# moble/scri

Measured on AMD Instinct MI355X. Metric: timesteps/sec for full BMS transform, l_max=16, 1e5 steps; fp64, higher is better.
Workload: dtype f64

## Files before the change

scri_amd/csrc/kernels_gemm_eval.hip:

```cpp
#include <cstdio>
#include <cstdlib>
#include <vector>

#include "kernels.h"

namespace bms {

typedef double v4d __attribute__((ext_vector_type(4)));

constexpr int E_BM = 64, E_BN = 64, E_KC = 8;
constexpr int E_PA = 10;
constexpr int E_PB = 64;
constexpr int E_ASZ = E_BM * E_PA;
constexpr int E_BSZ = E_KC * E_PB;
constexpr int E_PC = 33;

struct EvalArgs {
  const BsplineTable* table;
  const double* x;
  const double* skew_a;
  const double* skew_b;
  double tt;
  long long g0, n, i_lo, i_hi;
  double* out;
  long long ldo;
  int search_halfwidth;
  double inv_dx;
  double* side;
  long long side_ld;
  unsigned long long* stats;
  int dbg;
  unsigned long long* trace;
};

#if BMS_PROBES
#define EV_DBG(ev) ((ev).dbg)
#define EV_TRACE(ev) ((ev).trace)
#else
#define EV_DBG(ev) 0
#define EV_TRACE(ev) (static_cast<unsigned long long*>(nullptr))
#endif

__device__ __forceinline__ int eval_lower_bound(const double* __restrict__ bp, int n_i, double sa, double sb, double tt, double y,
                                                long long guess, int halfwidth) {
  auto ue = [&](int i) {
    const double xi = bp[i];
    return xi + (sa * (xi - tt) + sb);
  };
  int lo = 0, hi = n_i;
  if (halfwidth > 0) {
    long long a = guess - halfwidth, b = guess + halfwidth;
    if (a < 0) a = 0;
    if (b > n_i) b = n_i;
    if (a < b) {
      const bool ok_lo = (a == 0) || ue((int)a - 1) < y;
      const bool ok_hi = (b == n_i) || !(ue((int)b) < y);
      if (ok_lo && ok_hi) lo = (int)a, hi = (int)b;
    }
  }
  while (lo < hi) {
    const int mid = (lo + hi) >> 1;
    if (ue(mid) < y)
      lo = mid + 1;
    else
      hi = mid;
  }
  return lo;
}

__device__ __forceinline__ double2 eval_ld2(const double* p) { return *reinterpret_cast<const double2*>(p); }
__device__ __forceinline__ double2 eval_ld2(const double __attribute__((address_space(3))) * p) {
  typedef double v2d_t __attribute__((ext_vector_type(2)));
  const v2d_t v = *(const v2d_t __attribute__((address_space(3)))*)p;
  return double2{v.x, v.y};
}

struct EvalMarch {
  int jl, jl_end, jl_open, f_lo, f_hi, i, n_i;
  double sa, sb, tt;
  double* op;
  long long ldo;
};

template <bool INTERIOR, class SRC, class WIN>
__device__ __forceinline__ bool eval_march(EvalMarch& m, const SRC& src, WIN win, int dbg) {
  if (!src.has(m.i)) return false;
  double xi = src.samp(m.i);
  double sk = m.sa * (xi - m.tt) + m.sb;
  double ue = xi + sk;
  const double inf = __builtin_huge_val();
  double xhi = (!INTERIOR && m.jl >= m.jl_open) ? inf : src.knot(m.jl + 1);
  while (true) {
    if (!(ue < xhi)) {
      if (++m.jl >= m.jl_end) return true;
      xhi = (!INTERIOR && m.jl >= m.jl_open) ? inf : src.knot(m.jl + 1);
    }
    if (ue < xhi) {
      const auto tb = src.tab(m.jl);
      int fl = m.jl - 1;
      if (!INTERIOR) fl = fl < m.f_lo ? m.f_lo : (fl > m.f_hi ? m.f_hi : fl);
      const double2 q0 = win(fl, 0), q1 = win(fl, 1), q2 = win(fl, 2), q3 = win(fl, 3);
      const double t = (xi - src.knot(m.jl)) + sk;
      const double2 m0 = eval_ld2(tb + 0), m1 = eval_ld2(tb + 2), m2 = eval_ld2(tb + 4), m3 = eval_ld2(tb + 6);
      const double2 m4 = eval_ld2(tb + 8), m5 = eval_ld2(tb + 10), m6 = eval_ld2(tb + 12), m7 = eval_ld2(tb + 14);
      const double b0 = fma(fma(fma(m6.x, t, m4.x), t, m2.x), t, m0.x);
      const double b1 = fma(fma(fma(m6.y, t, m4.y), t, m2.y), t, m0.y);
      const double b2 = fma(fma(fma(m7.x, t, m5.x), t, m3.x), t, m1.x);
      const double b3 = fma(fma(fma(m7.y, t, m5.y), t, m3.y), t, m1.y);
      double2 v;
      v.x = fma(b3, q3.x, fma(b2, q2.x, fma(b1, q1.x, b0 * q0.x)));
      v.y = fma(b3, q3.y, fma(b2, q2.y, fma(b1, q1.y, b0 * q0.y)));
      if (!(dbg & 2)) *reinterpret_cast<double2*>(m.op) = v;
      m.op += m.ldo;
      if (++m.i >= m.n_i) return true;
      if (!src.has(m.i)) return false;
      xi = src.samp(m.i);
      sk = m.sa * (xi - m.tt) + m.sb;
      ue = xi + sk;
    }
  }
}

struct EvalFromGlobal {
  const EvalArgs& ev;
  const double* bp;
  long long kT;
  __device__ __forceinline__ double knot(int jl) const { return ev.x[kT + jl]; }
  __device__ __forceinline__ const double* tab(int jl) const { return ev.table[kT + jl].m; }
  __device__ __forceinline__ bool has(int) const { return true; }
  __device__ __forceinline__ double samp(int i) const { return bp[i]; }
};
constexpr int E_XS = 256;
typedef const double __attribute__((address_space(3))) * lds_cdp;
typedef const double2 __attribute__((address_space(3))) * lds_cd2p;
struct EvalFromLds {
  lds_cdp t_lds;
  lds_cdp xk_lds;
  lds_cdp xs_lds;
  int i_a;
  double inv_dx;
  __device__ __forceinline__ double knot(int jl) const { return xk_lds[jl]; }
  __device__ __forceinline__ lds_cdp tab(int jl) const { return t_lds + 16 * jl; }
  __device__ __forceinline__ bool has(int i) const { return (unsigned)(i - i_a) < (unsigned)E_XS; }
  __device__ __forceinline__ double samp(int i) const { return xs_lds[i - i_a]; }
  __device__ __forceinline__ int first(double y, double sa, double sb, double tt, int n_i) const {
    int lo = 0, hi = E_XS;
    if (inv_dx > 0.0) {
      const double z = (y - (sb - sa * tt)) / (1.0 + sa);
      const double gf = (z - xs_lds[0]) * inv_dx;
      int g = gf < 0.0 ? 0 : (gf > (double)(E_XS - 1) ? E_XS - 1 : (int)gf);
      const double xa = xs_lds[g], xb = xs_lds[g + 1 < E_XS ? g + 1 : E_XS - 1];
      const bool below = xa + (sa * (xa - tt) + sb) < y;
      const bool next_below = xb + (sa * (xb - tt) + sb) < y;
      if (below && !next_below && g + 1 < E_XS)
        lo = hi = g + 1;
      else if (!below && g > 0) {
        const double xc = xs_lds[g - 1];
        if (xc + (sa * (xc - tt) + sb) < y) lo = hi = g;
      }
    }
#pragma unroll
    for (int st = 0; st < 9; ++st) {
      const int mid = lo < hi ? (lo + hi) >> 1 : (lo < E_XS ? lo : E_XS - 1);
      const double xi = xs_lds[mid];
      if (lo < hi) {
        if (xi + (sa * (xi - tt) + sb) < y)
          lo = mid + 1;
        else
          hi = mid;
      }
    }
    if ((lo > 0 || i_a == 0) && (lo < E_XS || i_a + E_XS >= n_i)) return (i_a + lo) < n_i ? (i_a + lo) : n_i;
    return -1;
  }
};

__device__ __forceinline__ bool eval_launch_wide_window(const EvalArgs& ev) {
  return !(ev.inv_dx > 0.0) || (EV_DBG(ev) & 32) || (ev.search_halfwidth > 0 && 2 * ev.search_halfwidth + 72 <= E_XS);
}
__device__ __forceinline__ bool eval_tile_window(const EvalArgs& ev, long long kT, int rows, int n_i, double smin, double smax, double inv_dx, int* i_a) {
  if (eval_launch_wide_window(ev)) {
    const bool ok = ev.search_halfwidth > 0 && 2 * ev.search_halfwidth + 72 <= E_XS;
    long long ia = kT - ev.i_lo - ev.search_halfwidth - 2;
    ia = ia > n_i - 1 ? n_i - 1 : ia;
    *i_a = (int)(ia < 0 ? 0 : ia);
    return ok;
  }
  const double r_hi = smax * inv_dx, r_lo = smin * inv_dx;
  const double amax = fabs(r_hi) > fabs(r_lo) ? fabs(r_hi) : fabs(r_lo);
  if (!(amax < 1e8)) {
    *i_a = 0;
    return false;
  }
  const long long margin = 3 + (long long)(0.03 * amax);
  long long ia = kT - ev.i_lo - (long long)ceil(r_hi) - margin - 1;
  const long long ib = kT + rows - ev.i_lo - (long long)floor(r_lo) + margin + 1;
  const bool ok = ib - ia <= E_XS;
  ia = ia > n_i - 1 ? n_i - 1 : ia;
  *i_a = (int)(ia < 0 ? 0 : ia);
  return ok;
}
__device__ __forceinline__ void wave_min_max(double& mn, double& mx) {
#pragma unroll
  for (int d = 32; d >= 1; d >>= 1) {
    const double a = __shfl_xor(mn, d, 64), b = __shfl_xor(mx, d, 64);
    mn = a < mn ? a : mn;
    mx = b > mx ? b : mx;
  }
}

template <class WIN>
__device__ __forceinline__ void eval_windows(const EvalArgs& ev, const bool from_lds, const EvalFromLds lds, int col, double sa, double sb, long long kT,
                                             int fa, int fb, WIN win) {
  const long long n = ev.n;
  {
    const long long cap = n - 3 - kT;
    if (fb > cap) fb = (int)cap;
  }
  if (fa >= fb) return;
  constexpr int FAR = 1 << 24;
  EvalMarch m;
  m.f_lo = kT > FAR ? -FAR : (int)(-kT), m.f_hi = n - 4 - kT > FAR ? FAR : (int)(n - 4 - kT);
  m.jl_open = n - 2 - kT > FAR ? FAR : (int)(n - 2 - kT);
  m.jl = fa == m.f_lo ? m.f_lo : fa + 1;
  m.jl_end = fb - 1 == m.f_hi ? m.jl_open + 1 : fb + 1;
  m.sa = sa, m.sb = sb;
  m.n_i = (int)(ev.i_hi - ev.i_lo);
  m.tt = ev.tt;
  m.ldo = ev.ldo;
  const double* bp = ev.x + ev.i_lo;
  int i = -1;
  if (kT + m.jl == 0)
    i = 0;
  else if (from_lds)
    i = lds.first(lds.knot(m.jl), m.sa, m.sb, m.tt, m.n_i);
  if (i < 0) {
    if (from_lds && ev.stats) atomicAdd(ev.stats + 1, 1ull);
    i = eval_lower_bound(bp, m.n_i, m.sa, m.sb, m.tt, ev.x[kT + m.jl], kT + m.jl - ev.i_lo, ev.search_halfwidth);
  }
  if (i >= m.n_i) return;
  m.i = i;
  m.op = ev.out + 2LL * col + (long long)i * ev.ldo;
  const bool interior = fa > m.f_lo && fb - 1 < m.f_hi && fb + 1 < m.jl_open;
  if (from_lds && interior) {
    if (eval_march<true>(m, lds, win, EV_DBG(ev))) return;
  } else if (from_lds) {
    if (eval_march<false>(m, lds, win, EV_DBG(ev))) return;
  }
  if (from_lds && ev.stats) atomicAdd(ev.stats + 1, 1ull);
  eval_march<false>(m, EvalFromGlobal{ev, bp, kT}, win, EV_DBG(ev));
}

template <int ROW_STEP>
__global__ __launch_bounds__(256, 3) void zgemm3m_eval_kernel(const double* __restrict__ A, long long lda, const double* __restrict__ B,
                                                             long long ldb, long long M, int N, int K, int nbm, int nbn,
                                                             int st_rows_log2, const double* __restrict__ col_scale, EvalArgs ev) {
  __shared__ __attribute__((aligned(16))) double2 lds[2 * E_ASZ + 2 * E_BSZ];
  static_assert(sizeof(double2) * (2 * E_ASZ + 2 * E_BSZ) >= sizeof(double2) * E_BM * E_PC, "the parked half tile must fit the operand LDS");
  __shared__ __attribute__((aligned(16))) double t_lds[64 * 16];
  __shared__ __attribute__((aligned(16))) double xk_lds[64];
  __shared__ __attribute__((aligned(16))) double xs_lds[E_XS];
  __shared__ __attribute__((aligned(16))) double2 sk_lds[E_BN];
  __shared__ double win_lds[4];
  double2* As = lds;
  double2* Bs = lds + 2 * E_ASZ;

  const int b = blockIdx.x;
  const int xcd = b & 7;
  const int q = b >> 3;
  const int st_cols_log2 = 6 - st_rows_log2;
  const int nsn = (nbn + (1 << st_cols_log2) - 1) >> st_cols_log2;
  const int S = (q >> 6) * 8 + xcd;
  const int r = q & 63;
  const int bm = ((S / nsn) << st_rows_log2) + (r >> st_cols_log2);
  const int bn = ((S % nsn) << st_cols_log2) + (r & ((1 << st_cols_log2) - 1));
  if (bm >= nbm || bn >= nbn) return;
  const long long m0 = (long long)bm * ROW_STEP;
  const int n0 = bn * E_BN;
  unsigned long long tr_t0 = 0;
  if (EV_TRACE(ev)) tr_t0 = __builtin_readcyclecounter();
  const int tid = threadIdx.x;
  const int wave = __builtin_amdgcn_readfirstlane(tid >> 6), lane = tid & 63;
  const int wm = wave >> 1, wn = wave & 1;
  const int fi = lane & 15, fk = lane >> 4;

  const long long rows_valid = (M - m0) < E_BM ? (M - m0) : E_BM;
  const long long kT = ev.g0 + m0;
  const int n_i = (int)(ev.i_hi - ev.i_lo);
  if (tid < E_BN) {
    const int col = n0 + tid < N ? n0 + tid : N - 1;
    const double sa = ev.skew_a ? ev.skew_a[col] : 0.0, sb = ev.skew_b ? ev.skew_b[col] : 0.0;
    sk_lds[tid] = double2{sa, sb};
    if (!eval_launch_wide_window(ev)) {
      const double s0 = sa * (ev.x[kT] - ev.tt) + sb, s1 = sa * (ev.x[kT + rows_valid - 1] - ev.tt) + sb;
      double mn = s0 < s1 ? s0 : s1, mx = s0 < s1 ? s1 : s0;
      wave_min_max(mn, mx);
      if (tid == 0) win_lds[0] = mn, win_lds[1] = mx;
    }
    if (tid == 0) {
      const double span = ev.x[kT + rows_valid - 1] - ev.x[kT];
      win_lds[2] = (rows_valid > 1 && span > 0.0) ? (double)(rows_valid - 1) / span : ev.inv_dx;
    }
  }

  v4d p1[2][2], p2[2][2], p3[2][2];
#pragma unroll
  for (int i = 0; i < 2; ++i)
#pragma unroll
    for (int j = 0; j < 2; ++j) p1[i][j] = p2[i][j] = p3[i][j] = v4d{0.0, 0.0, 0.0, 0.0};

  const int a_row = tid >> 3, a_k = tid & 7;
  const int b_row = tid >> 6, b_col = tid & 63;
  const double* a_ptr = A + (m0 + a_row) * lda + 2 * a_k;
  const double* b_ptr = B + (long long)b_row * ldb + 2 * (n0 + b_col);
  const bool a_ok0 = (m0 + a_row) < M, a_ok1 = (m0 + a_row + 32) < M;
  const double2 zero2 = {0.0, 0.0};
  double2 ra0, ra1, rb0, rb1;
  const int nk = (K + E_KC - 1) / E_KC;

#define E_LOAD_GLOBAL(kt)                                                                      \
  {                                                                                            \
    const int k0 = (kt)*E_KC;                                                                  \
    const bool kok = (k0 + a_k) < K;                                                           \
    ra0 = (a_ok0 && kok) ? *reinterpret_cast<const double2*>(a_ptr + 2 * k0) : zero2;          \
    ra1 = (a_ok1 && kok) ? *reinterpret_cast<const double2*>(a_ptr + 32 * lda + 2 * k0) : zero2; \
    const double* bp_ = b_ptr + (long long)k0 * ldb;                                           \
    rb0 = *reinterpret_cast<const double2*>(bp_);                                              \
    rb1 = *reinterpret_cast<const double2*>(bp_ + 4 * ldb);                                    \
  }
#define E_STORE_LDS(buf)                                        \
  {                                                             \
    double2* as_w = As + (buf)*E_ASZ + a_row * E_PA + a_k;      \
    as_w[0] = ra0;                                              \
    as_w[32 * E_PA] = ra1;                                      \
    double2* bs_w = Bs + (buf)*E_BSZ + b_row * E_PB + b_col;    \
    bs_w[0] = rb0;                                              \
    bs_w[4 * E_PB] = rb1;                                       \
  }

  E_LOAD_GLOBAL(0);
  E_STORE_LDS(0);
  __syncthreads();
  int i_a;
  const bool wide = eval_launch_wide_window(ev);
  const bool from_lds = eval_tile_window(ev, kT, (int)rows_valid, n_i, wide ? 0.0 : win_lds[0], wide ? 0.0 : win_lds[1], win_lds[2], &i_a);
  if (!from_lds && tid == 0 && ev.stats) atomicAdd(ev.stats, 1ull);
  if (from_lds) {
    if (tid == 0) {
      const int i_b = i_a + E_XS - 1 < n_i - 1 ? i_a + E_XS - 1 : n_i - 1;
      const double span = ev.x[ev.i_lo + i_b] - ev.x[ev.i_lo + i_a];
      win_lds[3] = (ev.inv_dx > 0.0 && i_b > i_a && span > 0.0) ? (double)(i_b - i_a) / span : 0.0;
    }
    {
      long long row = tid >> 2;
      if (row > rows_valid - 1) row = rows_valid - 1;
      const double* src = ev.table[kT + row].m + 4 * (tid & 3);
      const double2 v0 = *reinterpret_cast<const double2*>(src), v1 = *reinterpret_cast<const double2*>(src + 2);
      double2* dst = reinterpret_cast<double2*>(t_lds + 16 * (tid >> 2) + 4 * (tid & 3));
      dst[0] = v0, dst[1] = v1;
    }
    if (tid < 64) {
      long long row = tid;
      if (row > rows_valid - 1) row = rows_valid - 1;
      xk_lds[tid] = ev.x[kT + row];
    }
    {
      int i = i_a + tid;
      if (i > n_i - 1) i = n_i - 1;
      xs_lds[tid] = ev.x[ev.i_lo + i];
    }
  }

  const bool narrow = n0 + 32 >= N;
  const int rbase = narrow ? wave * 16 : wm * 32, cbase = narrow ? 0 : wn * 32;
  const bool wave_has_columns = n0 + cbase < N;
  for (int kt = 0; kt < nk; ++kt) {
    const int buf = kt & 1;
    if (kt + 1 < nk) E_LOAD_GLOBAL(kt + 1);
    const double2* as = As + buf * E_ASZ + (rbase + fi) * E_PA + fk;
    const double2* bs = Bs + buf * E_BSZ + fk * E_PB + cbase + fi;
#pragma unroll
    for (int kk = 0; wave_has_columns && kk < E_KC / 4; ++kk) {
      const double2 a0 = as[kk * 4];
      const double2 b0 = bs[kk * 4 * E_PB], b1 = bs[kk * 4 * E_PB + 16];
      const double sa0 = a0.x + a0.y, sb0 = b0.x + b0.y, sb1 = b1.x + b1.y;
      p1[0][0] = __builtin_amdgcn_mfma_f64_16x16x4f64(a0.x, b0.x, p1[0][0], 0, 0, 0);
      p1[0][1] = __builtin_amdgcn_mfma_f64_16x16x4f64(a0.x, b1.x, p1[0][1], 0, 0, 0);
      p2[0][0] = __builtin_amdgcn_mfma_f64_16x16x4f64(a0.y, b0.y, p2[0][0], 0, 0, 0);
      p2[0][1] = __builtin_amdgcn_mfma_f64_16x16x4f64(a0.y, b1.y, p2[0][1], 0, 0, 0);
      p3[0][0] = __builtin_amdgcn_mfma_f64_16x16x4f64(sa0, sb0, p3[0][0], 0, 0, 0);
      p3[0][1] = __builtin_amdgcn_mfma_f64_16x16x4f64(sa0, sb1, p3[0][1], 0, 0, 0);
      if (!narrow) {
        const double2 a1 = as[16 * E_PA + kk * 4];
        const double sa1 = a1.x + a1.y;
        p1[1][0] = __builtin_amdgcn_mfma_f64_16x16x4f64(a1.x, b0.x, p1[1][0], 0, 0, 0);
        p1[1][1] = __builtin_amdgcn_mfma_f64_16x16x4f64(a1.x, b1.x, p1[1][1], 0, 0, 0);
        p2[1][0] = __builtin_amdgcn_mfma_f64_16x16x4f64(a1.y, b0.y, p2[1][0], 0, 0, 0);
        p2[1][1] = __builtin_amdgcn_mfma_f64_16x16x4f64(a1.y, b1.y, p2[1][1], 0, 0, 0);
        p3[1][0] = __builtin_amdgcn_mfma_f64_16x16x4f64(sa1, sb0, p3[1][0], 0, 0, 0);
        p3[1][1] = __builtin_amdgcn_mfma_f64_16x16x4f64(sa1, sb1, p3[1][1], 0, 0, 0);
      }
    }
    if (kt + 1 < nk) E_STORE_LDS(buf ^ 1);
    __syncthreads();
  }
#undef E_LOAD_GLOBAL
#undef E_STORE_LDS

  unsigned long long tr_t1 = 0;
  if (EV_TRACE(ev)) tr_t1 = __builtin_readcyclecounter();
  double2 cv[2][2][4];
#pragma unroll
  for (int j = 0; j < 2; ++j) {
    const int col = n0 + cbase + j * 16 + fi;
    const bool okc = col < N;
    const double sc_r = (okc && col_scale) ? col_scale[2 * col] : 1.0, sc_i = (okc && col_scale) ? col_scale[2 * col + 1] : 1.0;
#pragma unroll
    for (int i = 0; i < 2; ++i)
#pragma unroll
      for (int rr = 0; rr < 4; ++rr) {
        const double re = p1[i][j][rr] - p2[i][j][rr];
        const double im = (p3[i][j][rr] - p1[i][j][rr]) - p2[i][j][rr];
        cv[i][j][rr] = double2{re * sc_r, im * sc_i};
      }
  }
  double2* Cs = lds;
  const int ec = tid & 31, eg = tid >> 5;
#pragma unroll
  for (int h = 0; h < 2; ++h) {
    if (narrow ? h == 0 : wn == h) {
#pragma unroll
      for (int j = 0; j < 2; ++j)
#pragma unroll
        for (int i = 0; i < 2; ++i)
#pragma unroll
          for (int rr = 0; rr < 4; ++rr)
            if (i == 0 || !narrow) Cs[(rbase + i * 16 + fk + 4 * rr) * E_PC + j * 16 + fi] = cv[i][j][rr];
    }
    __syncthreads();
    const int col = n0 + h * 32 + ec;
    if (col < N && !(EV_DBG(ev) & 1)) {
      if (ROW_STEP == 64 && ev.side != nullptr && eg < 6) {
        const int row = eg < 3 ? eg : 58 + eg;
        if (row < rows_valid) *reinterpret_cast<double2*>(ev.side + ((long long)bm * 6 + eg) * ev.side_ld + 2LL * col) = Cs[row * E_PC + ec];
      }
      int fa = 8 * eg, fb = fa + 8;
      const int f_own = 61, f_rows = (int)rows_valid - 3;
      if (fb > f_own) fb = f_own;
      if (fb > f_rows) fb = f_rows;
      const auto win = [&](int fl, int qq) { return Cs[(fl + qq) * E_PC + ec]; };
      const EvalFromLds src{(lds_cdp)t_lds, (lds_cdp)xk_lds, (lds_cdp)xs_lds, i_a, from_lds ? win_lds[3] : 0.0};
      const double2 sk = sk_lds[h * 32 + ec];
      eval_windows(ev, from_lds, src, col, sk.x, sk.y, kT, fa, fb, win);
    }
    if (h == 0) __syncthreads();
  }
  if (EV_TRACE(ev) && tid == 0) {
    const unsigned hw = __builtin_amdgcn_s_getreg((31 << 11) | 4), xcc = __builtin_amdgcn_s_getreg((31 << 11) | 20);
    unsigned long long* tp = ev.trace + 5LL * b;
    tp[0] = (unsigned long long)hw | ((unsigned long long)xcc << 32);
    tp[1] = (unsigned long long)bm | ((unsigned long long)bn << 32);
    tp[2] = tr_t0, tp[3] = tr_t1, tp[4] = __builtin_readcyclecounter();
  }
}

__global__ __launch_bounds__(64) void spline_straddle_eval_kernel(int N, int n_row_tiles, int n_col_panels, EvalArgs ev, long long M) {
  __shared__ __attribute__((aligned(16))) double2 w_lds[6][64];
  __shared__ __attribute__((aligned(16))) double t_lds[8 * 16];
  __shared__ __attribute__((aligned(16))) double xk_lds[8];
  __shared__ __attribute__((aligned(16))) double xs_lds[E_XS];
  const int tid = threadIdx.x;
  const int bnd = blockIdx.x / n_col_panels;
  const int col = (blockIdx.x - bnd * n_col_panels) * 64 + tid;
  if (bnd + 1 >= n_row_tiles) return;
  const long long kT = ev.g0 + 64LL * bnd + 61;
  const int n_i = (int)(ev.i_hi - ev.i_lo);
  const long long k_last = ev.g0 + M - 1;
  const int colc = col < N ? col : N - 1;
  const double sa_t = ev.skew_a ? ev.skew_a[colc] : 0.0, sb_t = ev.skew_b ? ev.skew_b[colc] : 0.0;
  double smin = 0.0, smax = 0.0;
  if (!eval_launch_wide_window(ev)) {
    const double s0 = sa_t * (ev.x[kT] - ev.tt) + sb_t, s1 = sa_t * (ev.x[kT + 5 > k_last ? k_last : kT + 5] - ev.tt) + sb_t;
    smin = s0 < s1 ? s0 : s1, smax = s0 < s1 ? s1 : s0;
    wave_min_max(smin, smax);
  }
  double inv_dx_loc = ev.inv_dx;
  {
    const long long ka = kT - 29 < ev.g0 ? ev.g0 : kT - 29, kb = kT + 34 > k_last ? k_last : kT + 34;
    const double span = ev.x[kb] - ev.x[ka];
    if (kb > ka && span > 0.0) inv_dx_loc = (double)(kb - ka) / span;
  }
  int i_a;
  const bool from_lds = eval_tile_window(ev, kT, 6, n_i, smin, smax, inv_dx_loc, &i_a);
  if (!from_lds && tid == 0 && ev.stats) atomicAdd(ev.stats, 1ull);
  double inv_dx_win = 0.0;
  if (from_lds) {
    {
      const int i_b = i_a + E_XS - 1 < n_i - 1 ? i_a + E_XS - 1 : n_i - 1;
      const double span = ev.x[ev.i_lo + i_b] - ev.x[ev.i_lo + i_a];
      if (ev.inv_dx > 0.0 && i_b > i_a && span > 0.0) inv_dx_win = (double)(i_b - i_a) / span;
    }
    {
      long long jj = kT + (tid >> 3);
      if (jj > k_last) jj = k_last;
      reinterpret_cast<double2*>(t_lds)[tid] = *reinterpret_cast<const double2*>(ev.table[jj].m + 2 * (tid & 7));
    }
    if (tid < 8) {
      long long jj = kT + tid;
      if (jj > k_last) jj = k_last;
      xk_lds[tid] = ev.x[jj];
    }
#pragma unroll
    for (int r = 0; r < E_XS / 64; ++r) {
      int i = i_a + tid + 64 * r;
      if (i > n_i - 1) i = n_i - 1;
      xs_lds[tid + 64 * r] = ev.x[ev.i_lo + i];
    }
    __syncthreads();
  }
  if (col >= N) return;
  int fb = 3;
  {
    const long long f_rows = ev.g0 + M - 3 - kT;
    if (fb > f_rows) fb = (int)f_rows;
  }
  const double* s0 = ev.side + ((long long)bnd * 6 + 3) * ev.side_ld + 2LL * col;
  const double* s1 = ev.side + ((long long)(bnd + 1) * 6 + 0) * ev.side_ld + 2LL * col;
#pragma unroll
  for (int e = 0; e < 3; ++e) {
    w_lds[e][tid] = *reinterpret_cast<const double2*>(s0 + e * ev.side_ld);
    w_lds[3 + e][tid] = *reinterpret_cast<const double2*>(s1 + e * ev.side_ld);
  }
  const auto win = [&](int fl, int qq) { return w_lds[fl + qq][tid]; };
  const EvalFromLds src{(lds_cdp)t_lds, (lds_cdp)xk_lds, (lds_cdp)xs_lds, i_a, inv_dx_win};
  eval_windows(ev, from_lds, src, col, sa_t, sb_t, kT, 0, fb, win);
}

hipError_t launch_zgemm3m_eval(hipStream_t stream, const double* A, long long lda, const double* B, long long ldb, long long M, int N,
                               int K, const double* col_scale, const SplineEval& e) {
  if (M <= 0 || N <= 0 || e.i_hi <= e.i_lo) return hipSuccess;
  if (M < 4) return hipErrorInvalidValue;
  EvalArgs ev;
  ev.table = e.table, ev.x = e.x, ev.skew_a = e.skew_a, ev.skew_b = e.skew_b, ev.tt = e.tt, ev.g0 = e.g0, ev.n = e.n_knots;
  ev.i_lo = e.i_lo, ev.i_hi = e.i_hi, ev.out = e.out, ev.ldo = e.ldo, ev.search_halfwidth = e.search_halfwidth;
  ev.inv_dx = e.inv_dx;
  ev.side = e.side, ev.side_ld = e.side_ld;
  ev.stats = e.stats;
  ev.dbg = 0;
#if BMS_PROBES
  static const int dbg_env = BMS_PROBE_ENV("SCRI_AMD_GEMM_EVAL_DBG") ? atoi(BMS_PROBE_ENV("SCRI_AMD_GEMM_EVAL_DBG")) : 0;
  ev.dbg = dbg_env;
#endif
  const int step = (e.step == 61 || e.step == 64) ? e.step : (e.side ? 64 : 61);
  if (step == 64 && !e.side) return hipErrorInvalidValue;
  if (step == 61) ev.side = nullptr;
  const int nbm = step == 61 ? (int)((M - 3 + 60) / 61) : (int)((M + 63) / 64);
  const int nbn = (N + E_BN - 1) / E_BN;
  static const int st_env = BMS_PROBE_ENV("SCRI_AMD_ZGEMM_ST_ROWS_LOG2") ? atoi(BMS_PROBE_ENV("SCRI_AMD_ZGEMM_ST_ROWS_LOG2")) : -1;
  const int st_rows_log2 = (st_env >= 0 && st_env <= 6) ? st_env : (nbm >= 512 ? 6 : 5);
  const int sr = 1 << st_rows_log2, sc = 64 >> st_rows_log2;
  const long long n_super = (long long)((nbm + sr - 1) / sr) * ((nbn + sc - 1) / sc);
  const long long grid = ((n_super + 7) / 8) * 8 * 64;
  ev.trace = nullptr;
#if BMS_PROBES
  const char* trace_path = BMS_PROBE_ENV("SCRI_AMD_GEMM_EVAL_TRACE");
  if (trace_path) {
    if (hipMalloc(&ev.trace, 40 * (size_t)grid) != hipSuccess) ev.trace = nullptr;
    if (ev.trace) (void)hipMemsetAsync(ev.trace, 0, 40 * (size_t)grid, stream);
  }
#endif
  if (step == 61)
    hipLaunchKernelGGL(zgemm3m_eval_kernel<61>, dim3((unsigned)grid), dim3(256), 0, stream, A, lda, B, ldb, M, N, K, nbm, nbn, st_rows_log2,
                       col_scale, ev);
  else {
    hipLaunchKernelGGL(zgemm3m_eval_kernel<64>, dim3((unsigned)grid), dim3(256), 0, stream, A, lda, B, ldb, M, N, K, nbm, nbn, st_rows_log2,
                       col_scale, ev);
    const long long n_straddle = (long long)(nbm - 1) * nbn;
    if (n_straddle > 0x7fffffffLL) return hipErrorInvalidValue;
    if (nbm > 1 && !(EV_DBG(ev) & 4))
      hipLaunchKernelGGL(spline_straddle_eval_kernel, dim3((unsigned)n_straddle), dim3(64), 0, stream, N, nbm, nbn, ev, M);
  }
#if BMS_PROBES
  if (ev.trace) {
    std::vector<unsigned long long> h(5 * (size_t)grid);
    (void)hipStreamSynchronize(stream);
    (void)hipMemcpy(h.data(), ev.trace, 40 * (size_t)grid, hipMemcpyDeviceToHost);
    (void)hipFree(ev.trace);
    if (FILE* f = fopen(trace_path, "wb")) {
      fwrite(h.data(), 8, h.size(), f);
      fclose(f);
    }
  }
#endif
  return hipGetLastError();
}

long long zgemm3m_eval_side_rows(long long M) { return 6 * ((M + 63) / 64); }

}
```

Measured before the change: 19.07 million.

## Micro-optimize fused zgemm-eval kernel: buffer loads, precomputed reciprocals, magic division

Bundles several micro-optimizations into the fused GEMM+spline-eval kernel. Global tile loads move to raw buffer loads with out-of-bounds zeroing in place of per-lane predicated loads, and the k-loop is unrolled by two. Per-column 1/(1+sa) is precomputed and stored in LDS, the binary search is skipped when no lane needs it (wave ballot), and the superblock div/mod uses a host-computed magic multiplier. The tile window computation moves into the prologue on thread 0 and is broadcast with readfirstlane. These changes add launch-time stride checks and rely on buffer OOB semantics being correct for the tails.

```diff
diff --git a/scri_amd/csrc/kernels_gemm_eval.hip b/scri_amd/csrc/kernels_gemm_eval.hip
--- a/scri_amd/csrc/kernels_gemm_eval.hip
+++ b/scri_amd/csrc/kernels_gemm_eval.hip
@@ -143,10 +143,10 @@
   __device__ __forceinline__ lds_cdp tab(int jl) const { return t_lds + 16 * jl; }
   __device__ __forceinline__ bool has(int i) const { return (unsigned)(i - i_a) < (unsigned)E_XS; }
   __device__ __forceinline__ double samp(int i) const { return xs_lds[i - i_a]; }
-  __device__ __forceinline__ int first(double y, double sa, double sb, double tt, int n_i) const {
+  __device__ __forceinline__ int first(double y, double sa, double sb, double tt, double rinv, int n_i) const {
     int lo = 0, hi = E_XS;
     if (inv_dx > 0.0) {
-      const double z = (y - (sb - sa * tt)) / (1.0 + sa);
+      const double z = (y - (sb - sa * tt)) * rinv;
       const double gf = (z - xs_lds[0]) * inv_dx;
       int g = gf < 0.0 ? 0 : (gf > (double)(E_XS - 1) ? E_XS - 1 : (int)gf);
       const double xa = xs_lds[g], xb = xs_lds[g + 1 < E_XS ? g + 1 : E_XS - 1];
@@ -159,15 +159,17 @@
         if (xc + (sa * (xc - tt) + sb) < y) lo = hi = g;
       }
     }
-#pragma unroll
-    for (int st = 0; st < 9; ++st) {
-      const int mid = lo < hi ? (lo + hi) >> 1 : (lo < E_XS ? lo : E_XS - 1);
-      const double xi = xs_lds[mid];
-      if (lo < hi) {
-        if (xi + (sa * (xi - tt) + sb) < y)
-          lo = mid + 1;
-        else
-          hi = mid;
+    if (__builtin_amdgcn_ballot_w64(lo < hi) != 0) {
+#pragma unroll
+      for (int st = 0; st < 9; ++st) {
+        const int mid = lo < hi ? (lo + hi) >> 1 : (lo < E_XS ? lo : E_XS - 1);
+        const double xi = xs_lds[mid];
+        if (lo < hi) {
+          if (xi + (sa * (xi - tt) + sb) < y)
+            lo = mid + 1;
+          else
+            hi = mid;
+        }
       }
     }
     if ((lo > 0 || i_a == 0) && (lo < E_XS || i_a + E_XS >= n_i)) return (i_a + lo) < n_i ? (i_a + lo) : n_i;
@@ -210,8 +212,8 @@
 }
 
 template <class WIN>
-__device__ __forceinline__ void eval_windows(const EvalArgs& ev, const bool from_lds, const EvalFromLds lds, int col, double sa, double sb, long long kT,
-                                             int fa, int fb, WIN win) {
+__device__ __forceinline__ void eval_windows(const EvalArgs& ev, const bool from_lds, const EvalFromLds lds, int col, double sa, double sb, double rinv,
+                                             long long kT, int fa, int fb, WIN win) {
   const long long n = ev.n;
   {
     const long long cap = n - 3 - kT;
@@ -233,7 +235,7 @@
   if (kT + m.jl == 0)
     i = 0;
   else if (from_lds)
-    i = lds.first(lds.knot(m.jl), m.sa, m.sb, m.tt, m.n_i);
+    i = lds.first(lds.knot(m.jl), m.sa, m.sb, m.tt, rinv, m.n_i);
   if (i < 0) {
     if (from_lds && ev.stats) atomicAdd(ev.stats + 1, 1ull);
     i = eval_lower_bound(bp, m.n_i, m.sa, m.sb, m.tt, ev.x[kT + m.jl], kT + m.jl - ev.i_lo, ev.search_halfwidth);
@@ -254,14 +256,16 @@
 template <int ROW_STEP>
 __global__ __launch_bounds__(256, 3) void zgemm3m_eval_kernel(const double* __restrict__ A, long long lda, const double* __restrict__ B,
                                                              long long ldb, long long M, int N, int K, int nbm, int nbn,
-                                                             int st_rows_log2, const double* __restrict__ col_scale, EvalArgs ev) {
+                                                             int st_rows_log2, unsigned nsn_magic, const double* __restrict__ col_scale, EvalArgs ev) {
   __shared__ __attribute__((aligned(16))) double2 lds[2 * E_ASZ + 2 * E_BSZ];
   static_assert(sizeof(double2) * (2 * E_ASZ + 2 * E_BSZ) >= sizeof(double2) * E_BM * E_PC, "the parked half tile must fit the operand LDS");
   __shared__ __attribute__((aligned(16))) double t_lds[64 * 16];
   __shared__ __attribute__((aligned(16))) double xk_lds[64];
   __shared__ __attribute__((aligned(16))) double xs_lds[E_XS];
   __shared__ __attribute__((aligned(16))) double2 sk_lds[E_BN];
-  __shared__ double win_lds[4];
+  __shared__ __attribute__((aligned(16))) double rc_lds[E_BN];
+  __shared__ double win_lds[1];
+  __shared__ int wini_lds[2];
   double2* As = lds;
   double2* Bs = lds + 2 * E_ASZ;
 
@@ -272,8 +276,10 @@
   const int nsn = (nbn + (1 << st_cols_log2) - 1) >> st_cols_log2;
   const int S = (q >> 6) * 8 + xcd;
   const int r = q & 63;
-  const int bm = ((S / nsn) << st_rows_log2) + (r >> st_cols_log2);
-  const int bn = ((S % nsn) << st_cols_log2) + (r & ((1 << st_cols_log2) - 1));
+  unsigned s_q = __umulhi((unsigned)S, nsn_magic), s_r = (unsigned)S - s_q * (unsigned)nsn;
+  if (s_r >= (unsigned)nsn) ++s_q, s_r -= (unsigned)nsn;
+  const int bm = (int)(s_q << st_rows_log2) + (r >> st_cols_log2);
+  const int bn = (int)(s_r << st_cols_log2) + (r & ((1 << st_cols_log2) - 1));
   if (bm >= nbm || bn >= nbn) return;
   const long long m0 = (long long)bm * ROW_STEP;
   const int n0 = bn * E_BN;
@@ -291,15 +297,27 @@
     const int col = n0 + tid < N ? n0 + tid : N - 1;
     const double sa = ev.skew_a ? ev.skew_a[col] : 0.0, sb = ev.skew_b ? ev.skew_b[col] : 0.0;
     sk_lds[tid] = double2{sa, sb};
+    rc_lds[tid] = 1.0 / (1.0 + sa);
+    double mn = 0.0, mx = 0.0;
     if (!eval_launch_wide_window(ev)) {
       const double s0 = sa * (ev.x[kT] - ev.tt) + sb, s1 = sa * (ev.x[kT + rows_valid - 1] - ev.tt) + sb;
-      double mn = s0 < s1 ? s0 : s1, mx = s0 < s1 ? s1 : s0;
+      mn = s0 < s1 ? s0 : s1, mx = s0 < s1 ? s1 : s0;
       wave_min_max(mn, mx);
-      if (tid == 0) win_lds[0] = mn, win_lds[1] = mx;
     }
     if (tid == 0) {
       const double span = ev.x[kT + rows_valid - 1] - ev.x[kT];
-      win_lds[2] = (rows_valid > 1 && span > 0.0) ? (double)(rows_valid - 1) / span : ev.inv_dx;
+      const double inv_dx_tile = (rows_valid > 1 && span > 0.0) ? (double)(rows_valid - 1) / span : ev.inv_dx;
+      int ia;
+      const bool ok = eval_tile_window(ev, kT, (int)rows_valid, n_i, mn, mx, inv_dx_tile, &ia);
+      double inv_dx_win = 0.0;
+      if (ok) {
+        const int i_b = ia + E_XS - 1 < n_i - 1 ? ia + E_XS - 1 : n_i - 1;
+        const double wspan = ev.x[ev.i_lo + i_b] - ev.x[ev.i_lo + ia];
+        inv_dx_win = (ev.inv_dx > 0.0 && i_b > ia && wspan > 0.0) ? (double)(i_b - ia) / wspan : 0.0;
+      } else if (ev.stats)
+        atomicAdd(ev.stats, 1ull);
+      win_lds[0] = inv_dx_win;
+      wini_lds[0] = ia, wini_lds[1] = ok ? 1 : 0;
     }
   }
 
@@ -311,46 +329,42 @@
 
   const int a_row = tid >> 3, a_k = tid & 7;
   const int b_row = tid >> 6, b_col = tid & 63;
-  const double* a_ptr = A + (m0 + a_row) * lda + 2 * a_k;
-  const double* b_ptr = B + (long long)b_row * ldb + 2 * (n0 + b_col);
-  const bool a_ok0 = (m0 + a_row) < M, a_ok1 = (m0 + a_row + 32) < M;
-  const double2 zero2 = {0.0, 0.0};
+  const int nk = (K + E_KC - 1) / E_KC;
+  constexpr int E_OOB = 0x7ffffff0;
+  const double* a_base = A + m0 * lda;
+  const double* b_base = B + 2LL * n0;
+  const long long a_bytes = ((rows_valid - 1) * lda + 2LL * K) * 8;
+  const int b_bytes = (int)(((E_KC - 1) * ldb + 2LL * E_BN) * 8);
+  const int a_off0 = (int)(a_row * lda * 8) + 16 * a_k, a_off1 = a_off0 + (int)(32 * lda * 8);
+  const int b_off0 = (int)(b_row * ldb * 8) + 16 * b_col, b_off1 = b_off0 + (int)(4 * ldb * 8);
+  const bool k_tail = (nk - 1) * E_KC + a_k >= K;
+  const int a_off0_last = k_tail ? E_OOB : a_off0, a_off1_last = k_tail ? E_OOB : a_off1;
   double2 ra0, ra1, rb0, rb1;
-  const int nk = (K + E_KC - 1) / E_KC;
-
-#define E_LOAD_GLOBAL(kt)                                                                      \
-  {                                                                                            \
-    const int k0 = (kt)*E_KC;                                                                  \
-    const bool kok = (k0 + a_k) < K;                                                           \
-    ra0 = (a_ok0 && kok) ? *reinterpret_cast<const double2*>(a_ptr + 2 * k0) : zero2;          \
-    ra1 = (a_ok1 && kok) ? *reinterpret_cast<const double2*>(a_ptr + 32 * lda + 2 * k0) : zero2; \
-    const double* bp_ = b_ptr + (long long)k0 * ldb;                                           \
-    rb0 = *reinterpret_cast<const double2*>(bp_);                                              \
-    rb1 = *reinterpret_cast<const double2*>(bp_ + 4 * ldb);                                    \
-  }
-#define E_STORE_LDS(buf)                                        \
-  {                                                             \
-    double2* as_w = As + (buf)*E_ASZ + a_row * E_PA + a_k;      \
-    as_w[0] = ra0;                                              \
-    as_w[32 * E_PA] = ra1;                                      \
-    double2* bs_w = Bs + (buf)*E_BSZ + b_row * E_PB + b_col;    \
-    bs_w[0] = rb0;                                              \
-    bs_w[4 * E_PB] = rb1;                                       \
-  }
-
-  E_LOAD_GLOBAL(0);
-  E_STORE_LDS(0);
+  const auto load_global = [&](int kt, bool last) __attribute__((always_inline)) {
+    const auto a_rs = __builtin_amdgcn_make_buffer_rsrc(const_cast<double*>(a_base + 2 * E_KC * kt), 0, (int)(a_bytes - 16LL * E_KC * kt), 0x00020000);
+    const auto b_rs = __builtin_amdgcn_make_buffer_rsrc(const_cast<double*>(b_base + (long long)kt * E_KC * ldb), 0, b_bytes, 0x00020000);
+    ra0 = __builtin_bit_cast(double2, __builtin_amdgcn_raw_buffer_load_b128(a_rs, last ? a_off0_last : a_off0, 0, 0));
+    ra1 = __builtin_bit_cast(double2, __builtin_amdgcn_raw_buffer_load_b128(a_rs, last ? a_off1_last : a_off1, 0, 0));
+    rb0 = __builtin_bit_cast(double2, __builtin_amdgcn_raw_buffer_load_b128(b_rs, b_off0, 0, 0));
+    rb1 = __builtin_bit_cast(double2, __builtin_amdgcn_raw_buffer_load_b128(b_rs, b_off1, 0, 0));
+  };
+  double2* const as_w0 = As + a_row * E_PA + a_k;
+  double2* const bs_w0 = Bs + b_row * E_PB + b_col;
+  const auto store_lds = [&](int buf) __attribute__((always_inline)) {
+    double2* as_w = as_w0 + buf * E_ASZ;
+    as_w[0] = ra0;
+    as_w[32 * E_PA] = ra1;
+    double2* bs_w = bs_w0 + buf * E_BSZ;
+    bs_w[0] = rb0;
+    bs_w[4 * E_PB] = rb1;
+  };
+
+  load_global(0, nk == 1);
+  store_lds(0);
   __syncthreads();
-  int i_a;
-  const bool wide = eval_launch_wide_window(ev);
-  const bool from_lds = eval_tile_window(ev, kT, (int)rows_valid, n_i, wide ? 0.0 : win_lds[0], wide ? 0.0 : win_lds[1], win_lds[2], &i_a);
-  if (!from_lds && tid == 0 && ev.stats) atomicAdd(ev.stats, 1ull);
+  const int i_a = __builtin_amdgcn_readfirstlane(wini_lds[0]);
+  const bool from_lds = __builtin_amdgcn_readfirstlane(wini_lds[1]) != 0;
   if (from_lds) {
-    if (tid == 0) {
-      const int i_b = i_a + E_XS - 1 < n_i - 1 ? i_a + E_XS - 1 : n_i - 1;
-      const double span = ev.x[ev.i_lo + i_b] - ev.x[ev.i_lo + i_a];
-      win_lds[3] = (ev.inv_dx > 0.0 && i_b > i_a && span > 0.0) ? (double)(i_b - i_a) / span : 0.0;
-    }
     {
       long long row = tid >> 2;
       if (row > rows_valid - 1) row = rows_valid - 1;
@@ -374,11 +388,12 @@
   const bool narrow = n0 + 32 >= N;
   const int rbase = narrow ? wave * 16 : wm * 32, cbase = narrow ? 0 : wn * 32;
   const bool wave_has_columns = n0 + cbase < N;
-  for (int kt = 0; kt < nk; ++kt) {
-    const int buf = kt & 1;
-    if (kt + 1 < nk) E_LOAD_GLOBAL(kt + 1);
-    const double2* as = As + buf * E_ASZ + (rbase + fi) * E_PA + fk;
-    const double2* bs = Bs + buf * E_BSZ + fk * E_PB + cbase + fi;
+  const double2* const as_r0 = As + (rbase + fi) * E_PA + fk;
+  const double2* const bs_r0 = Bs + fk * E_PB + cbase + fi;
+  const auto turn = [&](int kt, int buf, bool more, bool last) __attribute__((always_inline)) {
+    if (more) load_global(kt + 1, last);
+    const double2* as = as_r0 + buf * E_ASZ;
+    const double2* bs = bs_r0 + buf * E_BSZ;
 #pragma unroll
     for (int kk = 0; wave_has_columns && kk < E_KC / 4; ++kk) {
       const double2 a0 = as[kk * 4];
@@ -401,11 +416,15 @@
         p3[1][1] = __builtin_amdgcn_mfma_f64_16x16x4f64(sa1, sb1, p3[1][1], 0, 0, 0);
       }
     }
-    if (kt + 1 < nk) E_STORE_LDS(buf ^ 1);
+    if (more) store_lds(buf ^ 1);
     __syncthreads();
-  }
-#undef E_LOAD_GLOBAL
-#undef E_STORE_LDS
+  };
+  int kt = 0;
+  for (; kt + 3 < nk; kt += 2) {
+    turn(kt, 0, true, false);
+    turn(kt + 1, 1, true, false);
+  }
+  for (; kt < nk; ++kt) turn(kt, kt & 1, kt + 1 < nk, kt + 2 == nk);
 
   unsigned long long tr_t1 = 0;
   if (EV_TRACE(ev)) tr_t1 = __builtin_readcyclecounter();
@@ -449,9 +468,9 @@
       if (fb > f_own) fb = f_own;
       if (fb > f_rows) fb = f_rows;
       const auto win = [&](int fl, int qq) { return Cs[(fl + qq) * E_PC + ec]; };
-      const EvalFromLds src{(lds_cdp)t_lds, (lds_cdp)xk_lds, (lds_cdp)xs_lds, i_a, from_lds ? win_lds[3] : 0.0};
+      const EvalFromLds src{(lds_cdp)t_lds, (lds_cdp)xk_lds, (lds_cdp)xs_lds, i_a, win_lds[0]};
       const double2 sk = sk_lds[h * 32 + ec];
-      eval_windows(ev, from_lds, src, col, sk.x, sk.y, kT, fa, fb, win);
+      eval_windows(ev, from_lds, src, col, sk.x, sk.y, rc_lds[h * 32 + ec], kT, fa, fb, win);
     }
     if (h == 0) __syncthreads();
   }
@@ -478,6 +497,7 @@
   const long long k_last = ev.g0 + M - 1;
   const int colc = col < N ? col : N - 1;
   const double sa_t = ev.skew_a ? ev.skew_a[colc] : 0.0, sb_t = ev.skew_b ? ev.skew_b[colc] : 0.0;
+  const double rinv_t = 1.0 / (1.0 + sa_t);
   double smin = 0.0, smax = 0.0;
   if (!eval_launch_wide_window(ev)) {
     const double s0 = sa_t * (ev.x[kT] - ev.tt) + sb_t, s1 = sa_t * (ev.x[kT + 5 > k_last ? k_last : kT + 5] - ev.tt) + sb_t;
@@ -533,13 +553,14 @@
   }
   const auto win = [&](int fl, int qq) { return w_lds[fl + qq][tid]; };
   const EvalFromLds src{(lds_cdp)t_lds, (lds_cdp)xk_lds, (lds_cdp)xs_lds, i_a, inv_dx_win};
-  eval_windows(ev, from_lds, src, col, sa_t, sb_t, kT, 0, fb, win);
+  eval_windows(ev, from_lds, src, col, sa_t, sb_t, rinv_t, kT, 0, fb, win);
 }
 
 hipError_t launch_zgemm3m_eval(hipStream_t stream, const double* A, long long lda, const double* B, long long ldb, long long M, int N,
                                int K, const double* col_scale, const SplineEval& e) {
   if (M <= 0 || N <= 0 || e.i_hi <= e.i_lo) return hipSuccess;
   if (M < 4) return hipErrorInvalidValue;
+  if (lda < 2LL * K || lda * 8 * E_BM >= 0x7ffffff0LL || ldb * 8 * E_KC + 16LL * E_BN >= 0x7ffffff0LL) return hipErrorInvalidValue;
   EvalArgs ev;
   ev.table = e.table, ev.x = e.x, ev.skew_a = e.skew_a, ev.skew_b = e.skew_b, ev.tt = e.tt, ev.g0 = e.g0, ev.n = e.n_knots;
   ev.i_lo = e.i_lo, ev.i_hi = e.i_hi, ev.out = e.out, ev.ldo = e.ldo, ev.search_halfwidth = e.search_halfwidth;
@@ -561,6 +582,8 @@
   const int sr = 1 << st_rows_log2, sc = 64 >> st_rows_log2;
   const long long n_super = (long long)((nbm + sr - 1) / sr) * ((nbn + sc - 1) / sc);
   const long long grid = ((n_super + 7) / 8) * 8 * 64;
+  const unsigned nsn = (unsigned)((nbn + sc - 1) / sc);
+  const unsigned nsn_magic = nsn == 1 ? 0xffffffffu : (unsigned)(0x100000000ULL / nsn);
   ev.trace = nullptr;
 #if BMS_PROBES
   const char* trace_path = BMS_PROBE_ENV("SCRI_AMD_GEMM_EVAL_TRACE");
@@ -571,10 +594,10 @@
 #endif
   if (step == 61)
     hipLaunchKernelGGL(zgemm3m_eval_kernel<61>, dim3((unsigned)grid), dim3(256), 0, stream, A, lda, B, ldb, M, N, K, nbm, nbn, st_rows_log2,
-                       col_scale, ev);
+                       nsn_magic, col_scale, ev);
   else {
     hipLaunchKernelGGL(zgemm3m_eval_kernel<64>, dim3((unsigned)grid), dim3(256), 0, stream, A, lda, B, ldb, M, N, K, nbm, nbn, st_rows_log2,
-                       col_scale, ev);
+                       nsn_magic, col_scale, ev);
     const long long n_straddle = (long long)(nbm - 1) * nbn;
     if (n_straddle > 0x7fffffffLL) return hipErrorInvalidValue;
     if (nbm > 1 && !(EV_DBG(ev) & 4))
```

Result: faster. 21.39 million, median of 6 (+12.2%).
